# Chang-Tun-Yu/HLS-final-Visual-Odometry

Measured on AMD Instinct MI355X. Metric: stereo frame-pairs/sec (detect+match), KITTI 1241x376; matches bit-exact, higher is better.
Workload: dtype u8; 1 GPU; KITTI 1241x376 stereo quad-match (prev/curr x L/R), default 50x50 bins; noise=0, gpu_max_hw_queues=4, streams_per_gpu=256, frames_in_hbm=8, parallelism=1x independent stream groups

## Files before the change

### hls-final-visual-odometry_amd/csrc/kernels_match.hip

```cpp
#include "vh_findmatch.h"
#include "vh_wave.h"
#include <algorithm>
#include <cstdlib>
#include <type_traits>

#ifdef VH_FLOW_STATS
__device__ unsigned long long g_flow_stats[12];
extern "C" int32_t vh_debug_flow_stats(unsigned long long *out, int32_t reset) {
  if (hipMemcpyFromSymbol(out, HIP_SYMBOL(g_flow_stats), sizeof(g_flow_stats)) != hipSuccess) return -3;
  if (reset) { unsigned long long z[12] = {0}; if (hipMemcpyToSymbol(HIP_SYMBOL(g_flow_stats), z, sizeof(z)) != hipSuccess) return -3; }
  return 0;
}
#define VH_STAT(k, n) do { if ((threadIdx.x & 63) == 0) atomicAdd(&g_flow_stats[k], (unsigned long long)(n)); } while (0)
#else
#define VH_STAT(k, n) do { } while (0)
#endif

#ifndef VH_MATCH_WAVES
#define VH_MATCH_WAVES 7
#endif

namespace {

template <bool MAX>
__device__ __forceinline__ int32_t row16_allreduce(int32_t v) {
#define VH_ROW_STEP(CTRL)                                                                   \
  {                                                                                         \
    const int32_t t = __builtin_amdgcn_update_dpp(v, v, CTRL, 0xF, 0xF, false);             \
    v = MAX ? max(v, t) : min(v, t);                                                        \
  }
  VH_ROW_STEP(0x128)
  VH_ROW_STEP(0x124)
  VH_ROW_STEP(0x122)
  VH_ROW_STEP(0x121)
#undef VH_ROW_STEP
  return v;
}

template <class T>
__device__ __forceinline__ T ld_off(const T *base, uint32_t byte_off) { return *(const T *)((const char *)base + byte_off); }
template <class T>
__device__ __forceinline__ void st_off(T *base, uint32_t byte_off, T x) { *(T *)((char *)base + byte_off) = x; }
template <class T>
__device__ __forceinline__ T ld_uniform(const T *p) { return *(const __attribute__((address_space(4))) T *)(uintptr_t)p; }
__device__ __forceinline__ int32_t ld_uniform_i32(const int32_t *p) { return __builtin_amdgcn_readfirstlane(ld_uniform(p)); }

template <bool TESTED, class First, class Step>
__device__ __forceinline__ void walk_columns(const VhSets &s, const int32_t *__restrict__ cbs, int32_t c, int32_t UB0, int32_t UB1, int32_t VB0,
                                             int32_t VB1, int32_t ULO_MAX, int32_t UHI_MIN, int32_t VA0, int32_t VA1, First first, Step step) {
  const int32_t lane = threadIdx.x & 63;
  const bool merged = !TESTED && VB0 == 0 && VB1 == s.vbn - 1;
  const int32_t UB1w = merged ? UB0 : UB1;
  for (int32_t cb = UB0; cb <= UB1w; cb += 64) {
    const int32_t ncb = min(64, UB1w - cb + 1);
    int32_t t_p0 = 0, t_p1 = 0, t_a0 = 0, t_a1 = 0;
    if (lane < ncb) {
      const int32_t row = (c * s.ubn + cb + lane) * s.vbn;
      t_p0 = ld_off(cbs, (uint32_t)(row + VB0) * 4u);
      t_p1 = ld_off(cbs, (uint32_t)(merged ? (c * s.ubn + UB1 + 1) * s.vbn : row + VB1 + 1) * 4u);
      if (TESTED) {
        const int32_t ubx = cb + lane;
        const bool in_ = ubx * s.binsize >= ULO_MAX && ubx * s.binsize + s.binsize - 1 <= UHI_MIN;
        t_a0 = in_ ? ((VA0 <= VA1) ? cbs[row + VA0] : t_p1) : 1;
        t_a1 = in_ ? ((VA0 <= VA1) ? cbs[row + VA1 + 1] : t_p1) : 0;
      }
    }
    int32_t ci = -1, pc = -64, p1 = 0;
    const auto advance = [&]() -> bool {
      pc += 64;
      while (pc >= p1) {
        if (++ci >= ncb) return false;
        pc = __builtin_amdgcn_readlane(t_p0, ci); p1 = __builtin_amdgcn_readlane(t_p1, ci);
      }
      return true;
    };
    if (!advance()) continue;
    first(pc, p1);
    for (;;) {
      const int32_t c_pc = pc, c_p1 = p1, c_ci = ci;
      const bool more = advance();
      int32_t pa0 = 1, pa1 = 0;
      if (TESTED) { pa0 = __builtin_amdgcn_readlane(t_a0, c_ci); pa1 = __builtin_amdgcn_readlane(t_a1, c_ci); }
      step(c_pc, c_p1, pa0, pa1, more, pc, p1);
      if (!more) break;
    }
  }
}

template <bool TESTED, bool NEED_UV, class Consume>
__device__ __forceinline__ void walk_region(const VhSets &s, const int32_t *__restrict__ cbs, const uint32_t *__restrict__ cuv,
                                            const uint4 *__restrict__ cdesc, int32_t c, int32_t UB0, int32_t UB1, int32_t VB0,
                                            int32_t VB1, int32_t ULO_MAX, int32_t UHI_MIN, int32_t VA0, int32_t VA1,
                                            Consume consume) {
  const int32_t lane = threadIdx.x & 63;
  int32_t pl = 0;
  uint32_t gu = 0;
  uint4 g0, g1;
  const auto load = [&](int32_t pc, int32_t p1) __attribute__((always_inline)) {
    pl = min(pc + lane, p1 - 1);
    if (NEED_UV) gu = cuv[pl];
    g0 = cdesc[2 * (int64_t)pl]; g1 = cdesc[2 * (int64_t)pl + 1];
  };
  walk_columns<TESTED>(s, cbs, c, UB0, UB1, VB0, VB1, ULO_MAX, UHI_MIN, VA0, VA1, load,
    [&](int32_t pc, int32_t p1, int32_t pa0, int32_t pa1, bool more, int32_t npc, int32_t np1) __attribute__((always_inline)) {
      const int32_t c_pl = pl;
      const uint32_t c_gu = gu;
      const uint4 c_g0 = g0, c_g1 = g1;
      if (more) load(npc, np1);
      consume(pc, p1, pa0, pa1, c_pl, c_gu, c_g0, c_g1);
    });
}

__device__ __forceinline__ void glds16(const void *gbase, uint32_t byte_off, uint32_t lds_dst) {
  asm volatile("s_mov_b32 m0, %2\n\ts_nop 0\n\tglobal_load_lds_dwordx4 %0, %1" ::"v"(byte_off), "s"(gbase), "s"(lds_dst) : "memory");
}
__device__ __forceinline__ void glds4(const void *gbase, uint32_t byte_off, uint32_t lds_dst) {
  asm volatile("s_mov_b32 m0, %2\n\ts_nop 0\n\tglobal_load_lds_dword %0, %1" ::"v"(byte_off), "s"(gbase), "s"(lds_dst) : "memory");
}
__device__ __forceinline__ uint32_t lds_addr(const void *p) {
  return __builtin_amdgcn_readfirstlane((uint32_t)(uintptr_t)(const __attribute__((address_space(3))) void *)p);
}

template <bool TESTED, class Consume>
__device__ __forceinline__ void walk_region_lds(const VhSets &s, const int32_t *__restrict__ cbs, const uint32_t *__restrict__ cuv,
                                                const uint4 *__restrict__ cdesc, int32_t c, int32_t UB0, int32_t UB1, int32_t VB0,
                                                int32_t VB1, int32_t ULO_MAX, int32_t UHI_MIN, int32_t VA0, int32_t VA1,
                                                uint4 *wD, uint32_t *wU, Consume consume) {
  const uint32_t ldsD = lds_addr(wD), ldsU = lds_addr(wU);
  const uint32_t lane32 = (uint32_t)(threadIdx.x & 63) * 32u;
  const auto issue = [&](int32_t b, int32_t pc, int32_t p1) __attribute__((always_inline)) {
    const uint32_t off = min((uint32_t)pc * 32u + lane32, (uint32_t)(p1 - 1) * 32u);
    glds16(cdesc, off, ldsD + (uint32_t)b * 2048u); glds16(cdesc, off + 16u, ldsD + (uint32_t)b * 2048u + 1024u);
    if (TESTED) glds4(cuv, off >> 3, ldsU + (uint32_t)b * 256u);
  };
  int32_t buf = 0;
  walk_columns<TESTED>(s, cbs, c, UB0, UB1, VB0, VB1, ULO_MAX, UHI_MIN, VA0, VA1,
    [&](int32_t pc, int32_t p1) __attribute__((always_inline)) {
      asm volatile("s_waitcnt lgkmcnt(0)" ::: "memory");
      buf = 0;
      issue(0, pc, p1);
    },
    [&](int32_t pc, int32_t p1, int32_t pa0, int32_t pa1, bool more, int32_t npc, int32_t np1) __attribute__((always_inline)) {
      const int32_t c_buf = buf;
      if (more) {
        buf ^= 1;
        asm volatile("s_waitcnt lgkmcnt(0)" ::: "memory");
        issue(buf, npc, np1);
        if (TESTED) asm volatile("s_waitcnt vmcnt(3)" ::: "memory");
        else asm volatile("s_waitcnt vmcnt(2)" ::: "memory");
      } else {
        asm volatile("s_waitcnt vmcnt(0)" ::: "memory");
      }
      consume(pc, p1, pa0, pa1, (const uint4 *)(wD + c_buf * 128), (const uint32_t *)(wU + c_buf * 64));
    });
}

__device__ __forceinline__ uint64_t tested_key_uniform_query(const uint32_t (&qd)[8], us2 lo2, us2 span2, uint32_t uv2,
                                                             const uint4 &b0, const uint4 &b1, uint32_t relpos) {
  const bool out = outside_window(uv2, lo2, span2);
  const uint32_t sad = sad32(make_uint4(qd[0], qd[1], qd[2], qd[3]), make_uint4(qd[4], qd[5], qd[6], qd[7]), b0, b1, 0);
  return out ? ~0ull : (((uint64_t)sad << 32) | relpos);
}

enum { KEY_HI16 = 0, KEY_W19 = 1, KEY_64 = 2 };
template <int KM> struct KeyT { typedef uint32_t type; };
template <> struct KeyT<KEY_64> { typedef uint64_t type; };
template <int KM>
__device__ __forceinline__ typename KeyT<KM>::type sad_key(const uint4 &a0, const uint4 &a1, const uint4 &b0, const uint4 &b1, uint32_t seed) {
  if (KM == KEY_HI16) return (typename KeyT<KM>::type)sad32<true>(a0, a1, b0, b1, seed);
  const uint32_t sad = sad32(a0, a1, b0, b1, 0);
  if (KM == KEY_W19) return (typename KeyT<KM>::type)((sad << 19) | seed);
  return (typename KeyT<KM>::type)(((uint64_t)sad << 32) | seed);
}
__device__ __forceinline__ int32_t key_mode_of(int32_t class_count, int32_t wide_keys) {
  if (class_count + 64 <= 0x10000 && !wide_keys) return KEY_HI16;
  return class_count <= VH_CLASS_POS_MAX && wide_keys < 2 ? KEY_W19 : KEY_64;
}

template <int Q, int P, int KM>
__device__ __forceinline__ int32_t join_phases(const typename KeyT<KM>::type (&best_key)[Q]) {
  static_assert(Q == 2 && P == 4, "the join splits the wave into two slots of two 16-lane rows");
  if (KM == KEY_64) {
    uint64_t k[Q];
#pragma unroll
    for (int32_t qi = 0; qi < Q; qi++) {
      k[qi] = (uint64_t)best_key[qi];
#pragma unroll
      for (int32_t d = 16; d < 64; d <<= 1) k[qi] = min(k[qi], vh_shfl_xor_u64(k[qi], d));
    }
    const uint64_t kk = (threadIdx.x & 32) ? k[1] : k[0];
    return kk == ~0ull ? -1 : (int32_t)(uint32_t)kk;
  }
  const auto h = __builtin_amdgcn_permlane32_swap((uint32_t)best_key[0], (uint32_t)best_key[1], false, false);
  const uint32_t kh = min(h[0], h[1]);
  const auto r = __builtin_amdgcn_permlane16_swap(kh, kh, false, false);
  const uint32_t k = min(r[0], r[1]);
  return k == 0xFFFFFFFFu ? -1 : (int32_t)(k & (KM == KEY_HI16 ? 0xFFFFu : 0x7FFFFu));
}

#ifndef VH_REDO_G
#define VH_REDO_G 2
#endif
struct RedoGroup {
  uint32_t qd[VH_REDO_G][8];
  us2 lo2[VH_REDO_G];
  int32_t lane[VH_REDO_G], n;
  int32_t umin, umax, vmin, vmax;
};
template <int Q>
__device__ __forceinline__ bool redo_take(uint64_t &todo, const uint4 (&a0)[Q], const uint4 (&a1)[Q], const uint32_t (&uv1)[Q],
                                          int32_t radius, int32_t rv, RedoGroup &g) {
  g.n = 0; g.umin = g.vmin = 0x7FFFFFFF; g.umax = g.vmax = -1;
#pragma unroll
  for (int32_t k = 0; k < VH_REDO_G; k++) {
    if (!todo) break;
    const int32_t fl = (int32_t)__builtin_ctzll(todo), fq = fl >> 5;
    todo &= todo - 1;
    uint4 x0 = a0[0], x1 = a1[0];
    uint32_t xu = uv1[0];
#pragma unroll
    for (int32_t qi = 1; qi < Q; qi++) if (fq == qi) { x0 = a0[qi]; x1 = a1[qi]; xu = uv1[qi]; }
    g.qd[k][0] = __builtin_amdgcn_readlane(x0.x, fl); g.qd[k][1] = __builtin_amdgcn_readlane(x0.y, fl);
    g.qd[k][2] = __builtin_amdgcn_readlane(x0.z, fl); g.qd[k][3] = __builtin_amdgcn_readlane(x0.w, fl);
    g.qd[k][4] = __builtin_amdgcn_readlane(x1.x, fl); g.qd[k][5] = __builtin_amdgcn_readlane(x1.y, fl);
    g.qd[k][6] = __builtin_amdgcn_readlane(x1.z, fl); g.qd[k][7] = __builtin_amdgcn_readlane(x1.w, fl);
    const uint32_t quv1 = __builtin_amdgcn_readlane(xu, fl);
    const int32_t u1 = (int32_t)(quv1 & 0xFFFF), v1 = (int32_t)(quv1 >> 16);
    g.lo2[k] = window_lo2(quv1, radius, rv);
    g.lane[k] = fl; g.n = k + 1;
    g.umin = min(g.umin, u1); g.umax = max(g.umax, u1); g.vmin = min(g.vmin, v1); g.vmax = max(g.vmax, v1);
  }
  return g.n > 0;
}

template <int Q> struct TileOut {
  int32_t wp;
  uint4 a0[Q], a1[Q];
  uint32_t uv1[Q];
  int32_t qpos[Q];
  bool valid[Q];
};

template <int Q, int P, bool SPEC, bool FLOW>
__device__ __forceinline__ void finish_tile(const VhSets &s, const VhMatchArgs &a, int32_t pass, int32_t stream, int32_t qset, int32_t cset,
                                            int32_t c, int32_t pbase, int32_t pcnt, const TileOut<Q> &o,
                                            int32_t *__restrict__ best, int32_t *__restrict__ redo_count) {
  static_assert(Q == 2 && P == 4, "one query per lane: slot lane >> 5, on the first 16-lane row of each half (join_phases)");
  const int32_t lane = threadIdx.x & 63;
  const uint32_t *__restrict__ cuv = s.s_uv + (int64_t)cset * s.cap;
  const uint4 *__restrict__ cdesc = (const uint4 *)(s.s_desc + (int64_t)cset * s.cap * 8);
  const int32_t *__restrict__ cbs = s.bin_start + (int64_t)cset * (s.nbins + 1);
  const int32_t rv = FLOW ? a.radius : a.disp_tol;
  const us2 span2 = window_span2(a.radius, rv);
  const int32_t *__restrict__ cidx = s.s_idx + (int64_t)cset * s.cap;
  const int32_t *__restrict__ qidx = s.s_idx + (int64_t)qset * s.cap;
  int32_t *__restrict__ tbl = best + ((int64_t)stream * 4 + a.pass[pass].slot) * s.cap;
  const bool hi = lane & 32;
  const bool mine = !(lane & 16) && (hi ? o.valid[1] : o.valid[0]);
  const uint32_t uv1 = hi ? o.uv1[1] : o.uv1[0];
  const int32_t qpos = hi ? o.qpos[1] : o.qpos[0];
  int32_t res = -1;
  bool fail = false;
  if (mine && o.wp >= 0) {
    int32_t wp = o.wp;
    VH_CHECK_RANGE(s, 7, wp, 0, pcnt);
    res = pbase + wp;
    if (SPEC) fail = outside_window(ld_off(cuv, (uint32_t)res * 4u), window_lo2(uv1, a.radius, rv), span2);
  }
  if (SPEC) {
    uint64_t todo = __ballot(fail);
    if (todo) {
      const int32_t nfail = (int32_t)__popcll(todo);
      VH_STAT(FLOW ? 7 : 10, nfail);
      if (lane == 0) atomicAdd(redo_count, nfail);
      RedoGroup g;
      while (redo_take<Q>(todo, o.a0, o.a1, o.uv1, a.radius, rv, g)) {
        uint64_t kk[VH_REDO_G];
#pragma unroll
        for (int32_t k = 0; k < VH_REDO_G; k++) kk[k] = ~0ull;
        if (FLOW) {
          const VhBins b = bins_of_interest(s, VhWindow{g.umin - a.radius, g.umax + a.radius, g.vmin - rv, g.vmax + rv});
          walk_region<false, true>(s, cbs, cuv, cdesc, c, b.ub0, b.ub1, b.vb0, b.vb1, 0, 0, 0, 0,
            [&](int32_t, int32_t, int32_t, int32_t, int32_t pl, uint32_t gu, const uint4 &g0, const uint4 &g1) {
#pragma unroll
              for (int32_t k = 0; k < VH_REDO_G; k++)
                if (k < g.n) kk[k] = min(kk[k], tested_key_uniform_query(g.qd[k], g.lo2[k], span2, gu, g0, g1, (uint32_t)(pl - pbase)));
            });
        } else {
          const int32_t *__restrict__ crs = s.row_start + (int64_t)cset * (4 * s.H + 1);
          const int32_t *__restrict__ cpos = s.r_pos + (int64_t)cset * s.cap;
          const int32_t x0 = ld_uniform_i32(crs + c * s.H + max(g.vmin - rv, 0));
          const int32_t x1 = ld_uniform_i32(crs + c * s.H + min(g.vmax + rv, s.H - 1) + 1);
          for (int32_t x = x0 + lane; x < x1; x += 64) {
            int32_t cp = cpos[x];
            VH_CHECK_RANGE(s, 3, cp, pbase, pbase + pcnt);
            const uint32_t gu = cuv[cp];
            const uint4 g0 = cdesc[2 * (int64_t)cp], g1 = cdesc[2 * (int64_t)cp + 1];
#pragma unroll
            for (int32_t k = 0; k < VH_REDO_G; k++)
              if (k < g.n) kk[k] = min(kk[k], tested_key_uniform_query(g.qd[k], g.lo2[k], span2, gu, g0, g1, (uint32_t)(cp - pbase)));
          }
        }
#pragma unroll
        for (int32_t k = 0; k < VH_REDO_G; k++)
          if (k < g.n) {
            const uint64_t kf = vh_wave_min_u64(kk[k]);
            int32_t wp = (int32_t)(uint32_t)kf;
            if (kf != ~0ull) VH_CHECK_RANGE(s, 7, wp, 0, pcnt);
            if (lane == g.lane[k]) res = kf == ~0ull ? -1 : pbase + wp;
          }
      }
    }
  }
  if (mine) st_off(tbl, (uint32_t)ld_off(qidx, (uint32_t)qpos * 4u) * 4u, res < 0 ? 0 : ld_off(cidx, (uint32_t)res * 4u));
}

struct FlowRegion {
  int32_t UB0, UB1, VB0, VB1;
  int32_t ULO_MAX, UHI_MIN, VA0, VA1;
};
template <int Q, int P, bool SPEC>
__device__ __forceinline__ FlowRegion flow_queries(const VhSets &s, const VhMatchArgs &a, int32_t rv, int32_t qset, int32_t q0, int32_t q1,
                                                   int32_t c, TileOut<Q> &out) {
  constexpr int L = 64 / P;
  static_assert(L == 8 || L == 16, "every 16-lane row must hold the whole tile (row-wise window reduction)");
  const int32_t l = (threadIdx.x & 63) % L;
  const uint32_t *__restrict__ quv = s.s_uv + (int64_t)qset * s.cap;
  const uint4 *__restrict__ qdesc = (const uint4 *)(s.s_desc + (int64_t)qset * s.cap * 8);
  bool (&valid)[Q] = out.valid;
  uint4 (&a0)[Q] = out.a0, (&a1)[Q] = out.a1;
  uint32_t (&uv1)[Q] = out.uv1;
  int32_t umin = 0x7FFFFFFF, umax = -1, vmin = 0x7FFFFFFF, vmax = -1;
  int32_t (&qp)[Q] = out.qpos;
  const int32_t *__restrict__ qsnake = s.snake_pos + (int64_t)qset * s.cap;
#pragma unroll
  for (int32_t qi = 0; qi < Q; qi++) {
    const int32_t q = q0 + L * qi + l;
    valid[qi] = q < q1;
    qp[qi] = valid[qi] ? q : q0;
    if (VH_SNAKE) qp[qi] = ld_off(qsnake, (uint32_t)qp[qi] * 4u);
#ifdef VH_CHECK
    {
      const int32_t *qbs = s.bin_start + (int64_t)qset * (s.nbins + 1);
      VH_CHECK_RANGE(s, 14, qp[qi], qbs[c * s.ubn * s.vbn], qbs[(c + 1) * s.ubn * s.vbn]);
    }
#endif
  }
#pragma unroll
  for (int32_t qi = 0; qi < Q; qi++) {
    const int32_t ql = qp[qi];
    uv1[qi] = ld_off(quv, (uint32_t)ql * 4u);
    a0[qi] = ld_off(qdesc, (uint32_t)ql * 32u); a1[qi] = ld_off(qdesc, (uint32_t)ql * 32u + 16u);
    const int32_t u1 = uv1[qi] & 0xFFFF, v1 = uv1[qi] >> 16;
    umin = min(umin, u1); umax = max(umax, u1); vmin = min(vmin, v1); vmax = max(vmax, v1);
  }
  umin = __builtin_amdgcn_readfirstlane(row16_allreduce<false>(umin));
  umax = __builtin_amdgcn_readfirstlane(row16_allreduce<true>(umax));
  vmin = __builtin_amdgcn_readfirstlane(row16_allreduce<false>(vmin));
  vmax = __builtin_amdgcn_readfirstlane(row16_allreduce<true>(vmax));
  const VhBins ub = bins_of_interest(s, VhWindow{umin - a.radius, umax + a.radius, vmin - rv, vmax + rv});
  FlowRegion r;
  r.UB0 = ub.ub0; r.UB1 = ub.ub1; r.VB0 = ub.vb0; r.VB1 = ub.vb1;
  r.ULO_MAX = umax - a.radius; r.UHI_MIN = umin + a.radius;
  const int32_t VLO_MAX = vmax - rv, VHI_MIN = vmin + rv;
  r.VA0 = SPEC ? 0 : max(r.VB0, (max(VLO_MAX, 0) + s.binsize - 1) / s.binsize);
  r.VA1 = SPEC ? 0 : min(r.VB1, (VHI_MIN + 1) / s.binsize - 1);
  VH_STAT(0, 1); VH_STAT(5, q1 - q0); VH_STAT(6, r.UB1 - r.UB0 + 1);
  return r;
}

template <int Q, int P, int KM, bool SPEC>
__device__ __forceinline__ void flow_tile(const VhSets &s, const VhMatchArgs &a, int32_t rv, int32_t cset, int32_t c, const FlowRegion &r,
                                          int32_t pbase, uint4 *wD, uint32_t *wU, TileOut<Q> &out) {
  constexpr int L = 64 / P;
  constexpr int TRIP = 2 * P;
  const int32_t ph = (threadIdx.x & 63) / L;
  const uint32_t *__restrict__ cuv = s.s_uv + (int64_t)cset * s.cap;
  const uint4 *__restrict__ cdesc = (const uint4 *)(s.s_desc + (int64_t)cset * s.cap * 8);
  const int32_t *__restrict__ cbs = s.bin_start + (int64_t)cset * (s.nbins + 1);
  const uint4 (&a0)[Q] = out.a0, (&a1)[Q] = out.a1;
  typedef typename KeyT<KM>::type key_t;
  const key_t KNONE = (key_t)~(key_t)0;
  key_t best_key[Q];
  int32_t v_lo[Q];
  us2 lo2[Q];
#pragma unroll
  for (int32_t qi = 0; qi < Q; qi++) {
    v_lo[qi] = (int32_t)(out.uv1[qi] >> 16) - rv;
    lo2[qi] = window_lo2(out.uv1[qi], a.radius, rv);
    best_key[qi] = KNONE;
  }
  const us2 span2 = window_span2(a.radius, rv);

  auto make_key = [&](auto test, int32_t qi, uint32_t uv2, const uint4 &b0, const uint4 &b1, uint32_t seed) -> key_t {
    constexpr int TEST = decltype(test)::value;
    bool out = false;
    if (TEST == 2) {
      out = outside_window(uv2, lo2[qi], span2);
    } else if (TEST == 1) {
      out = (uint32_t)((int32_t)(uv2 >> 16) - v_lo[qi]) > (uint32_t)(2 * rv);
    }
    const key_t key = sad_key<KM>(a0[qi], a1[qi], b0, b1, seed);
    return (TEST != 0 && out) ? KNONE : key;
  };
  walk_region_lds<!SPEC>(s, cbs, cuv, cdesc, c, r.UB0, r.UB1, r.VB0, r.VB1, r.ULO_MAX, r.UHI_MIN, r.VA0, r.VA1, wD, wU,
    [&](int32_t pc, int32_t p1, int32_t pa0, int32_t pa1, const uint4 *cD, const uint32_t *cU) {
      VH_STAT(1, 1);
      const int32_t mcnt = min(64, p1 - pc);
      const int32_t jend = (mcnt + TRIP - 1) & ~(TRIP - 1);
      const uint4 *rd = cD + ph;
      const uint32_t *ru = cU + ph;
      uint32_t seedA = (uint32_t)(pc - pbase + ph), seedB = seedA + P;
      int32_t j = 0;
      auto trip = [&](auto test, int32_t o) {
        const uint4 dA0 = rd[o], dA1 = rd[o + 64], dB0 = rd[o + P], dB1 = rd[o + 64 + P];
        uint32_t uA = 0, uB = 0;
        if (decltype(test)::value != 0) { uA = ru[o]; uB = ru[o + P]; }
#pragma unroll
        for (int32_t qi = 0; qi < Q; qi++) {
          const key_t kA = make_key(test, qi, uA, dA0, dA1, seedA + (uint32_t)o), kB = make_key(test, qi, uB, dB0, dB1, seedB + (uint32_t)o);
          best_key[qi] = min(min(kA, kB), best_key[qi]);
        }
      };
      auto run = [&](auto test, int32_t jstop) {
        if (jstop > j) VH_STAT(2 + decltype(test)::value, (jstop - j) / TRIP);
        for (; j + 2 * TRIP <= jstop; j += 2 * TRIP) {
          trip(test, 0); trip(test, TRIP);
          rd += 2 * TRIP; ru += 2 * TRIP; seedA += 2 * TRIP; seedB += 2 * TRIP;
        }
        if (j < jstop) {
          trip(test, 0);
          j += TRIP; rd += TRIP; ru += TRIP; seedA += TRIP; seedB += TRIP;
        }
      };
      if (SPEC) {
        run(std::integral_constant<int, 0>{}, jend);
      } else if (pa0 <= pa1) {
        const int32_t ja = min((min(max(pa0 - pc, 0), mcnt) + TRIP - 1) & ~(TRIP - 1), jend);
        const int32_t jb = max(min(max(pa1 - pc, 0), mcnt) & ~(TRIP - 1), ja);
        run(std::integral_constant<int, 1>{}, ja);
        run(std::integral_constant<int, 0>{}, jb);
        run(std::integral_constant<int, 1>{}, jend);
      } else {
        run(std::integral_constant<int, 2>{}, jend);
      }
    });
  out.wp = join_phases<Q, P, KM>(best_key);
}

template <bool SPEC, bool FLOW, class Tile>
__device__ __forceinline__ void search_tile(const VhSets &s, const VhMatchArgs &a, int32_t pass, int32_t stream, int32_t qset, int32_t cset,
                                            int32_t c, int32_t *__restrict__ best, int32_t *__restrict__ redo_count,
                                            TileOut<VH_FLOW_Q> &out, Tile tile) {
  const int32_t *cbs = s.bin_start + (int64_t)cset * (s.nbins + 1);
  const int32_t pbase = ld_uniform_i32(cbs + c * s.ubn * s.vbn);
  const int32_t pend = ld_uniform_i32(cbs + (c + 1) * s.ubn * s.vbn);
  const int32_t km = key_mode_of(pend - pbase, a.wide_keys);
  if (km == KEY_HI16) tile(std::integral_constant<int, KEY_HI16>{}, pbase, pend - pbase);
  else if (km == KEY_W19) tile(std::integral_constant<int, KEY_W19>{}, pbase, pend - pbase);
  else tile(std::integral_constant<int, KEY_64>{}, pbase, pend - pbase);
  finish_tile<VH_FLOW_Q, VH_FLOW_P, SPEC, FLOW>(s, a, pass, stream, qset, cset, c, pbase, pend - pbase, out, best, redo_count);
}

template <bool SPEC>
__device__ __forceinline__ void flow_pass(const VhSets &s, const VhMatchArgs &a, int32_t pass, int32_t stream, int32_t qset,
                                          int32_t cset, uint4 *wD, uint32_t *wU, int32_t *__restrict__ best, int32_t *__restrict__ redo_count) {
  const int32_t ntile = ld_uniform_i32(s.tile_cnt + qset);
  for (int32_t tile = __builtin_amdgcn_readfirstlane(blockIdx.x * 4 + (threadIdx.x >> 6)); tile < ntile;
       tile += gridDim.x * 4) {
    typedef int32_t i32x4 __attribute__((ext_vector_type(4)));
    const i32x4 t = ld_uniform((const i32x4 *)(s.tiles + (int64_t)qset * s.max_tiles + tile));
    const int32_t q0 = __builtin_amdgcn_readfirstlane(t.x), q1 = __builtin_amdgcn_readfirstlane(t.y);
    const int32_t c = __builtin_amdgcn_readfirstlane(t.z);
    TileOut<VH_FLOW_Q> out;
    const int32_t rv = a.pass[pass].flow ? a.radius : a.disp_tol;
    const FlowRegion r = flow_queries<VH_FLOW_Q, VH_FLOW_P, SPEC>(s, a, rv, qset, q0, q1, c, out);
    search_tile<SPEC, true>(s, a, pass, stream, qset, cset, c, best, redo_count, out,
      [&](auto km, int32_t pbase, int32_t) __attribute__((always_inline)) {
        flow_tile<VH_FLOW_Q, VH_FLOW_P, decltype(km)::value, SPEC>(s, a, rv, cset, c, r, pbase, wD, wU, out);
      });
  }
}

template <int Q, int P, int KM, bool SPEC>
__device__ __forceinline__ void rows_tile(const VhSets &s, const VhMatchArgs &a, int32_t pass, int32_t stream, int32_t qset,
                                          int32_t cset, int32_t q0, int32_t q1, int32_t c, int32_t pbase, int32_t pcnt, uint4 *wD,
                                          uint32_t *wU, uint32_t *wV, TileOut<Q> &out) {
  constexpr int L = 64 / P;
  static_assert(L == 8 || L == 16, "every 16-lane row must hold the whole tile");
  constexpr int TRIP = 2 * P;
  const int32_t lane = threadIdx.x & 63, ph = lane / L, l = lane % L;
  const int32_t nrow = 4 * s.H;
  const int32_t *__restrict__ crs = s.row_start + (int64_t)cset * (nrow + 1);
  const int32_t *__restrict__ qpos = s.r_pos + (int64_t)qset * s.cap;
  const uint32_t *__restrict__ quv = s.s_uv + (int64_t)qset * s.cap;
  const uint4 *__restrict__ qdesc = (const uint4 *)(s.s_desc + (int64_t)qset * s.cap * 8);
  const int32_t *__restrict__ cpos = s.r_pos + (int64_t)cset * s.cap;
  const uint32_t *__restrict__ cuv = s.s_uv + (int64_t)cset * s.cap;
  const uint4 *__restrict__ cdesc = (const uint4 *)(s.s_desc + (int64_t)cset * s.cap * 8);

  bool (&valid)[Q] = out.valid;
  uint4 (&a0)[Q] = out.a0, (&a1)[Q] = out.a1;
  uint32_t (&uv1)[Q] = out.uv1;
  int32_t (&qp)[Q] = out.qpos;
  typedef typename KeyT<KM>::type key_t;
  key_t best_key[Q];
  us2 lo2[Q];
  const us2 span2 = window_span2(a.radius, a.disp_tol);
  int32_t vmin = 0x7FFFFFFF, vmax = -1;
#pragma unroll
  for (int32_t qi = 0; qi < Q; qi++) {
    const int32_t q = q0 + L * qi + l;
    valid[qi] = q < q1;
    qp[qi] = ld_off(qpos, (uint32_t)(valid[qi] ? q : q0) * 4u);
    VH_CHECK_RANGE(s, 1, qp[qi], 0, s.cap);
    uv1[qi] = ld_off(quv, (uint32_t)qp[qi] * 4u);
    a0[qi] = ld_off(qdesc, (uint32_t)qp[qi] * 32u); a1[qi] = ld_off(qdesc, (uint32_t)qp[qi] * 32u + 16u);
    const int32_t v1 = uv1[qi] >> 16;
    lo2[qi] = window_lo2(uv1[qi], a.radius, a.disp_tol);
    best_key[qi] = (key_t)~(key_t)0;
    vmin = min(vmin, v1); vmax = max(vmax, v1);
  }
  vmin = __builtin_amdgcn_readfirstlane(row16_allreduce<false>(vmin));
  vmax = __builtin_amdgcn_readfirstlane(row16_allreduce<true>(vmax));
  VH_STAT(8, 1); VH_STAT(11, q1 - q0);
  const int32_t VLO = max(vmin - a.disp_tol, 0), VHI = min(vmax + a.disp_tol, s.H - 1);
  const int32_t r0 = ld_uniform_i32(crs + c * s.H + VLO);
  const int32_t r1 = ld_uniform_i32(crs + c * s.H + VHI + 1);
  for (int32_t rc = r0; rc < r1; rc += 64) {
    const int32_t mcnt = min(64, r1 - rc);
    int32_t cp = ld_off(cpos, (uint32_t)min(rc + lane, r1 - 1) * 4u);
    VH_CHECK_RANGE(s, 2, cp, pbase, pbase + pcnt);
    const uint4 g0 = ld_off(cdesc, (uint32_t)cp * 32u), g1 = ld_off(cdesc, (uint32_t)cp * 32u + 16u);
    uint32_t gu = 0;
    if (!SPEC) gu = ld_off(cuv, (uint32_t)cp * 4u);
    asm volatile("s_waitcnt lgkmcnt(0)" ::: "memory");
    wD[lane] = g0; wD[64 + lane] = g1; wU[lane] = (uint32_t)(cp - pbase);
    if (!SPEC) wV[lane] = gu;
    asm volatile("s_waitcnt lgkmcnt(0)" ::: "memory");
    const int32_t jend = (mcnt + TRIP - 1) & ~(TRIP - 1);
    VH_STAT(9, jend / TRIP);
    const uint4 *rd = wD + ph;
    const uint32_t *ru = wU + ph, *rv = wV + ph;
    for (int32_t j = 0; j < jend; j += TRIP) {
      const uint4 dA0 = rd[0], dA1 = rd[64], dB0 = rd[P], dB1 = rd[64 + P];
      const uint32_t sA = ru[0], sB = ru[P];
      uint32_t uA = 0, uB = 0;
      if (!SPEC) { uA = rv[0]; uB = rv[P]; }
#pragma unroll
      for (int32_t qi = 0; qi < Q; qi++) {
        key_t kA = sad_key<KM>(a0[qi], a1[qi], dA0, dA1, sA), kB = sad_key<KM>(a0[qi], a1[qi], dB0, dB1, sB);
        if (!SPEC) {
          kA = outside_window(uA, lo2[qi], span2) ? (key_t)~(key_t)0 : kA;
          kB = outside_window(uB, lo2[qi], span2) ? (key_t)~(key_t)0 : kB;
        }
        best_key[qi] = min(min(kA, kB), best_key[qi]);
      }
      rd += TRIP; ru += TRIP; rv += TRIP;
    }
  }
  out.wp = join_phases<Q, P, KM>(best_key);
}

template <bool SPEC>
__device__ __forceinline__ void rows_pass(const VhSets &s, const VhMatchArgs &a, int32_t pass, int32_t stream, int32_t qset,
                                          int32_t cset, uint4 *wD, uint32_t *wU, uint32_t *wV, int32_t *__restrict__ best, int32_t *__restrict__ redo_count) {
  const int32_t nrow = 4 * s.H;
  const int32_t *__restrict__ qrs = s.row_start + (int64_t)qset * (nrow + 1);
  int32_t cls_q0[5];
#pragma unroll
  for (int32_t c = 0; c <= 4; c++) cls_q0[c] = ld_uniform_i32(qrs + c * s.H);
  constexpr int T = VH_TILE_Q;
  for (int32_t tile = __builtin_amdgcn_readfirstlane(blockIdx.x * 4 + (threadIdx.x >> 6));; tile += gridDim.x * 4) {
    int32_t c = -1, q0 = 0, q1 = 0, t = tile;
#pragma unroll
    for (int32_t k = 0; k < 4; k++) {
      const int32_t nt = (cls_q0[k + 1] - cls_q0[k] + T - 1) / T;
      if (c < 0 && t < nt) { c = k; q0 = cls_q0[k] + T * t; q1 = min(cls_q0[k + 1], q0 + T); }
      if (c < 0) t -= nt;
    }
    if (c < 0) break;
    TileOut<VH_FLOW_Q> out;
    search_tile<SPEC, false>(s, a, pass, stream, qset, cset, c, best, redo_count, out,
      [&](auto km, int32_t pbase, int32_t pcnt) __attribute__((always_inline)) {
        rows_tile<VH_FLOW_Q, VH_FLOW_P, decltype(km)::value, SPEC>(s, a, pass, stream, qset, cset, q0, q1, c, pbase, pcnt, wD, wU, wV, out);
      });
  }
}

template <bool SPEC>
__global__ void __launch_bounds__(256) __attribute__((amdgpu_waves_per_eu(VH_MATCH_WAVES, 8)))
match_kernel(VhSets s, VhMatchArgs a, int32_t *__restrict__ best, int32_t *__restrict__ redo) {
  __shared__ uint4 sDesc[4 * 256];
  __shared__ uint32_t sAux[4 * 128];
  __shared__ uint32_t sAux2[SPEC ? 1 : 4 * 64];
  const int32_t pass = blockIdx.y, stream = blockIdx.z;
  if (a.prior && pass == 1) return;
#ifdef VH_EXP_SKIP
  if (VH_EXP_SKIP & (a.pass[pass].flow ? 2 : 1)) return;
#endif
  const int32_t qset = vh_row_set(a, stream, a.pass[pass].qset);
  const int32_t cset = vh_row_set(a, stream, a.pass[pass].cset);
  uint4 *wD = sDesc + (threadIdx.x >> 6) * 256;
  uint32_t *wU = sAux + (threadIdx.x >> 6) * 128;
  uint32_t *wV = sAux2 + (SPEC ? 0 : (threadIdx.x >> 6) * 64);
  int32_t *redo_count = redo + stream;
  if (a.pass[pass].flow) flow_pass<SPEC>(s, a, pass, stream, qset, cset, wD, wU, best, redo_count);
  else rows_pass<SPEC>(s, a, pass, stream, qset, cset, wD, wU, wV, best, redo_count);
}

}

void vh_launch_match(const VhSets &s, const VhMatchArgs &a, int32_t *best, int32_t *redo, int32_t speculative, int32_t grid_x,
                     int32_t lds_bytes, hipStream_t st) {
  if (!a.npass) return;
  VhMatchArgs m = a;
  static const int wide = [] { const char *e = getenv("VH_FLOW_WIDE_KEYS"); return e ? atoi(e) : 0; }();
  m.wide_keys = wide;
  static const int wgs = [] { const char *e = getenv("VH_FLOW_WGS"); return e ? atoi(e) : 0; }();
  static const int pad_env = [] { const char *e = getenv("VH_FLOW_LDS_PAD"); return e ? atoi(e) : -1; }();
  const int32_t gx = wgs > 0 ? wgs : (grid_x > 0 ? (grid_x | 1) : (((s.max_tiles + 3) / 4) | 1));
  dim3 grid(gx, m.npass, a.rows);
  static const size_t static_lds[2] = {
      [] { hipFuncAttributes at{}; return hipFuncGetAttributes(&at, (const void *)match_kernel<false>) == hipSuccess ? at.sharedSizeBytes : (size_t)0; }(),
      [] { hipFuncAttributes at{}; return hipFuncGetAttributes(&at, (const void *)match_kernel<true>) == hipSuccess ? at.sharedSizeBytes : (size_t)0; }()};
  const size_t have = static_lds[speculative ? 1 : 0];
  const int32_t pad = pad_env >= 0 ? pad_env : (wgs > 0 || grid_x <= 0 || lds_bytes <= 0 || have == 0 || (size_t)lds_bytes <= have ? 0 : (int32_t)((size_t)lds_bytes - have));
  if (speculative) hipLaunchKernelGGL(match_kernel<true>, grid, dim3(256), pad, st, s, m, best, redo);
  else hipLaunchKernelGGL(match_kernel<false>, grid, dim3(256), pad, st, s, m, best, redo);
}
```

Measured before the change: 119,500 pairs/s.

## Use chunk-local 16-bit keys with inline seeds and fully unroll the flow walk

Inside each 64-candidate chunk, the flow tile now builds compact 16-bit-position keys with seeds that are compile-time constants. Each chunk's minimum is promoted to the global key mode (HI16/W19/64-bit) once by adding the chunk base, instead of carrying wide keys and running seed adds per candidate. The variable-length trip loop is replaced by a fully unrolled per-chunk loop with a per-trip test-kind selection and a sched_barrier on full chunks. The none-detection changes to a floor compare, because rebased sentinel keys are no longer all-ones. The intent is to cut VALU work and 64-bit min operations in the inner SAD loop, at the cost of larger unrolled code and subtle sentinel handling.

```diff
diff --git a/hls-final-visual-odometry_amd/csrc/kernels_match.hip b/hls-final-visual-odometry_amd/csrc/kernels_match.hip
--- a/hls-final-visual-odometry_amd/csrc/kernels_match.hip
+++ b/hls-final-visual-odometry_amd/csrc/kernels_match.hip
@@ -172,6 +172,11 @@
   if (KM == KEY_W19) return (typename KeyT<KM>::type)((sad << 19) | seed);
   return (typename KeyT<KM>::type)(((uint64_t)sad << 32) | seed);
 }
+template <int KM>
+__device__ __forceinline__ typename KeyT<KM>::type key_none_floor() {
+  typedef typename KeyT<KM>::type key_t;
+  return KM == KEY_HI16 ? (key_t)0xFFFF0000u : KM == KEY_W19 ? (key_t)0xFFF80000u : (key_t)0x0000FFFF00000000ull;
+}
 __device__ __forceinline__ int32_t key_mode_of(int32_t class_count, int32_t wide_keys) {
   if (class_count + 64 <= 0x10000 && !wide_keys) return KEY_HI16;
   return class_count <= VH_CLASS_POS_MAX && wide_keys < 2 ? KEY_W19 : KEY_64;
@@ -189,13 +194,13 @@
       for (int32_t d = 16; d < 64; d <<= 1) k[qi] = min(k[qi], vh_shfl_xor_u64(k[qi], d));
     }
     const uint64_t kk = (threadIdx.x & 32) ? k[1] : k[0];
-    return kk == ~0ull ? -1 : (int32_t)(uint32_t)kk;
+    return kk >= key_none_floor<KEY_64>() ? -1 : (int32_t)(uint32_t)kk;
   }
   const auto h = __builtin_amdgcn_permlane32_swap((uint32_t)best_key[0], (uint32_t)best_key[1], false, false);
   const uint32_t kh = min(h[0], h[1]);
   const auto r = __builtin_amdgcn_permlane16_swap(kh, kh, false, false);
   const uint32_t k = min(r[0], r[1]);
-  return k == 0xFFFFFFFFu ? -1 : (int32_t)(k & (KM == KEY_HI16 ? 0xFFFFu : 0x7FFFFu));
+  return k >= key_none_floor<KM>() ? -1 : (int32_t)(k & (KM == KEY_HI16 ? 0xFFFFu : 0x7FFFFu));
 }
 
 #ifndef VH_REDO_G
@@ -374,6 +379,8 @@
                                           int32_t pbase, uint4 *wD, uint32_t *wU, TileOut<Q> &out) {
   constexpr int L = 64 / P;
   constexpr int TRIP = 2 * P;
+  constexpr int CH = 64 / TRIP;
+  static_assert(P * (2 * CH - 1) <= 64, "the chunk-local seeds P * k must be inline constants (integers up to 64)");
   const int32_t ph = (threadIdx.x & 63) / L;
   const uint32_t *__restrict__ cuv = s.s_uv + (int64_t)cset * s.cap;
   const uint4 *__restrict__ cdesc = (const uint4 *)(s.s_desc + (int64_t)cset * s.cap * 8);
@@ -392,7 +399,8 @@
   }
   const us2 span2 = window_span2(a.radius, rv);
 
-  auto make_key = [&](auto test, int32_t qi, uint32_t uv2, const uint4 &b0, const uint4 &b1, uint32_t seed) -> key_t {
+  constexpr uint32_t LNONE = 0xFFFF0000u;
+  auto make_key = [&](auto test, int32_t qi, uint32_t uv2, const uint4 &b0, const uint4 &b1, uint32_t seed) -> uint32_t {
     constexpr int TEST = decltype(test)::value;
     bool out = false;
     if (TEST == 2) {
@@ -400,50 +408,61 @@
     } else if (TEST == 1) {
       out = (uint32_t)((int32_t)(uv2 >> 16) - v_lo[qi]) > (uint32_t)(2 * rv);
     }
-    const key_t key = sad_key<KM>(a0[qi], a1[qi], b0, b1, seed);
-    return (TEST != 0 && out) ? KNONE : key;
+    const uint32_t key = sad_key<KEY_HI16>(a0[qi], a1[qi], b0, b1, seed);
+    return (TEST != 0 && out) ? LNONE : key;
+  };
+  auto global_key = [](uint32_t k, uint32_t vbase) -> key_t {
+    if (KM == KEY_HI16) return (key_t)(k + vbase);
+    const uint32_t pos = (k & 0xFFFFu) + vbase;
+    if (KM == KEY_W19) return (key_t)(((k & 0xFFFF0000u) << 3) | pos);
+    return (key_t)(((uint64_t)(k >> 16) << 32) | pos);
   };
   walk_region_lds<!SPEC>(s, cbs, cuv, cdesc, c, r.UB0, r.UB1, r.VB0, r.VB1, r.ULO_MAX, r.UHI_MIN, r.VA0, r.VA1, wD, wU,
     [&](int32_t pc, int32_t p1, int32_t pa0, int32_t pa1, const uint4 *cD, const uint32_t *cU) {
       VH_STAT(1, 1);
       const int32_t mcnt = min(64, p1 - pc);
-      const int32_t jend = (mcnt + TRIP - 1) & ~(TRIP - 1);
+      const int32_t nt = (mcnt + TRIP - 1) / TRIP;
       const uint4 *rd = cD + ph;
       const uint32_t *ru = cU + ph;
-      uint32_t seedA = (uint32_t)(pc - pbase + ph), seedB = seedA + P;
-      int32_t j = 0;
-      auto trip = [&](auto test, int32_t o) {
+      uint32_t cm[Q];
+      auto trip = [&](auto test, int32_t t) __attribute__((always_inline)) {
+        VH_STAT(2 + decltype(test)::value, 1);
+        const int32_t o = TRIP * t;
         const uint4 dA0 = rd[o], dA1 = rd[o + 64], dB0 = rd[o + P], dB1 = rd[o + 64 + P];
         uint32_t uA = 0, uB = 0;
         if (decltype(test)::value != 0) { uA = ru[o]; uB = ru[o + P]; }
 #pragma unroll
         for (int32_t qi = 0; qi < Q; qi++) {
-          const key_t kA = make_key(test, qi, uA, dA0, dA1, seedA + (uint32_t)o), kB = make_key(test, qi, uB, dB0, dB1, seedB + (uint32_t)o);
-          best_key[qi] = min(min(kA, kB), best_key[qi]);
+          const uint32_t kA = make_key(test, qi, uA, dA0, dA1, (uint32_t)o), kB = make_key(test, qi, uB, dB0, dB1, (uint32_t)(o + P));
+          cm[qi] = t == 0 ? min(kA, kB) : min(min(kA, kB), cm[qi]);
         }
       };
-      auto run = [&](auto test, int32_t jstop) {
-        if (jstop > j) VH_STAT(2 + decltype(test)::value, (jstop - j) / TRIP);
-        for (; j + 2 * TRIP <= jstop; j += 2 * TRIP) {
-          trip(test, 0); trip(test, TRIP);
-          rd += 2 * TRIP; ru += 2 * TRIP; seedA += 2 * TRIP; seedB += 2 * TRIP;
+      if (SPEC && nt == CH) {
+#pragma unroll
+        for (int32_t t = 0; t < CH; t++) {
+          trip(std::integral_constant<int, 0>{}, t);
+          if (t & 1) __builtin_amdgcn_sched_barrier(0);
         }
-        if (j < jstop) {
-          trip(test, 0);
-          j += TRIP; rd += TRIP; ru += TRIP; seedA += TRIP; seedB += TRIP;
+      } else if (SPEC || pa0 > pa1) {
+        constexpr int TEST = SPEC ? 0 : 2;
+#pragma unroll
+        for (int32_t t = 0; t < CH; t++) {
+          if (t >= nt) break;
+          trip(std::integral_constant<int, TEST>{}, t);
         }
-      };
-      if (SPEC) {
-        run(std::integral_constant<int, 0>{}, jend);
-      } else if (pa0 <= pa1) {
-        const int32_t ja = min((min(max(pa0 - pc, 0), mcnt) + TRIP - 1) & ~(TRIP - 1), jend);
-        const int32_t jb = max(min(max(pa1 - pc, 0), mcnt) & ~(TRIP - 1), ja);
-        run(std::integral_constant<int, 1>{}, ja);
-        run(std::integral_constant<int, 0>{}, jb);
-        run(std::integral_constant<int, 1>{}, jend);
       } else {
-        run(std::integral_constant<int, 2>{}, jend);
+        const int32_t ta = min((min(max(pa0 - pc, 0), mcnt) + TRIP - 1) / TRIP, nt);
+        const int32_t tb = max(min(max(pa1 - pc, 0), mcnt) / TRIP, ta);
+#pragma unroll
+        for (int32_t t = 0; t < CH; t++) {
+          if (t >= nt) break;
+          if (t >= ta && t < tb) trip(std::integral_constant<int, 0>{}, t);
+          else trip(std::integral_constant<int, 1>{}, t);
+        }
       }
+      const uint32_t vbase = (uint32_t)(pc - pbase + ph);
+#pragma unroll
+      for (int32_t qi = 0; qi < Q; qi++) best_key[qi] = min(best_key[qi], global_key(cm[qi], vbase));
     });
   out.wp = join_phases<Q, P, KM>(best_key);
 }
```

After: 122,800 pairs/s (median of 6 runs). 1.03x the previous value.
